# Soltanilara/av-aloha

Hardware: AMD Instinct MI355X
Metric: env-steps/sec (whole node) at 4096 parallel envs, SlotInsertion-3Arms (higher is better)
Workload: dtype f32

## Files before the change

### av_aloha_amd/csrc/avsim_phys.hip.h

```cpp
#pragma once
#include <hip/hip_runtime.h>

#include <cstddef>
#include <cstring>
#include <string>
#include <type_traits>
#include <vector>

#include "avsim_collide.hip.h"
#include "avsim_dev.h"
#include "avsim_math.hip.h"
#include "avsim_model.h"
#include "avsim_phys_layout.h"

namespace avs {

enum { J_FREE = 0, J_BALL = 1, J_SLIDE = 2, J_HINGE = 3 };
enum { R_EQ = 0, R_FLOSS = 1, R_LIMIT = 2, R_CONTACT = 3 };
constexpr int TREE_W = 8;
constexpr int ROW_W = 2 * TREE_W;
constexpr int ROW_S = ROW_W;
constexpr int CAND_MAX = 256;
constexpr int PROF_W = 26;
constexpr int NEAR_MAX = 512;
// ... 277 lines not shown
    const long long b = __builtin_bit_cast(long long, x);
    const unsigned lo = (unsigned)__builtin_amdgcn_readlane((int)(unsigned)b, l), hi = (unsigned)__builtin_amdgcn_readlane((int)(unsigned)(b >> 32), l);
    return __builtin_bit_cast(double, ((long long)hi << 32) | (long long)lo);
}

constexpr int GRP_MAX = 6;
constexpr int GA_W = 64, GA_Q = 16, GA_QW = 6;
template <typename T> AVS_DEV T qdiv(T t, T d, T dinv) { return sizeof(T) == 4 ? t * dinv : t / d; }
AVS_DEV float qrsqrt(float x) { return __builtin_amdgcn_rsqf(x); }
AVS_DEV double qrsqrt(double x) { return 1.0 / sqrt(x); }
template <typename T> struct QTol;
template <> struct QTol<double> { static constexpr double abs = 1e-10, rel = 0.0; };
template <> struct QTol<float> { static constexpr float abs = 1e-10f, rel = 2e-6f; };

template <bool B> struct BoolTag { static constexpr bool value = B; };

template <typename real>
struct NoslipLead {
    LDS_PTR(const real) Minv;
    LDS_PTR(const int) tadr;
    LDS_PTR(const int) tnum;
    LDS_PTR(const int) floss_dof;
    LDS_PTR(int) dmap;
    LDS_PTR(int) prof;
    int tridiag;
    int ntree, nv, neq, nfloss, nlg;
};

typedef int nl_v4 __attribute__((ext_vector_type(4)));
#define NL_PARAMS nl_v4 nl_a_, nl_v4 nl_b_, nl_v4 nl_c_
// ... 1277 lines not shown
    }
    int l = latch ? latch[i] : 0;
    reward[i] = reward_from_flags(f, task_id, &l);
    if (latch) latch[i] = l;
}
#endif


template <typename real, int G, typename SPEC = GenericSpec>
struct Env {
    KRef<real, SPEC> ka;
    int env = 0;
    int diverged = 0;
    int nit_sum = 0, nit_max = 0;
    bool profiling = false;
    real* r;
    int* ii;
    int lane, grp;
    const real* lr;
    const int* li;
    long long t_broad = 0, t_narrow = 0;
    __device__ Env(KRef<real, SPEC> ka_, real* r_, int* i_, int lane_, int grp_, const real* lr_, const int* li_)
        : ka(ka_), r(r_), ii(i_), lane(lane_), grp(grp_), lr(lr_), li(li_) {}
    AVS_DEV const int* LI() const {
        const int* p = li;
        if constexpr (spec_fixed<SPEC>) p = lds_at<const int>((unsigned)(ka->mo.nreal * sizeof(real)));
        AVS_ASSUME_LDS(p);
        return p;
    }
    AVS_DEV const real* LR() const {
        const real* p = lr;
        if constexpr (spec_fixed<SPEC>) p = lds_at<const real>(0u);
        AVS_ASSUME_LDS(p);
        return p;
    }
    AVS_DEV int nobj_() const { if constexpr (spec_fixed<SPEC>) return SPEC::nobj; else return ka->m.nobj; }
    AVS_DEV int hull_ovf_() const { if constexpr (spec_fixed<SPEC>) return SPEC::hull_ovf; else return ka->m.hull_ovf; }
    AVS_DEV GArr<real> rows_() const { return glb_block((GLB_PTR(real))ka->m.rJ_glob, env, (unsigned)(ka->lay.gefc * ROW_S)); }
    AVS_DEV GArr<real> rowsB_() const { return glb_block((GLB_PTR(real))ka->m.rB_glob, env, (unsigned)(ka->lay.gefc * ROW_S)); }
    AVS_DEV GArr<real> coup_() const { return glb_block((GLB_PTR(real))ka->m.gA_glob, env, (unsigned)(ka->lay.ggrp * GA_W)); }
    AVS_DEV GArr<int> near_() const { return glb_block((GLB_PTR(int))ka->m.near_glob, env, (unsigned)NEAR_MAX); }
    AVS_DEV GArr<int> cand_() const { return glb_block((GLB_PTR(int))ka->m.cand_glob, env, (unsigned)CAND_MAX); }
    AVS_DEV GArr<real> bxo_() const { return glb_block((GLB_PTR(real))ka->m.bxo_glob, env, (unsigned)(64 * BOX_OVF_W)); }
    AVS_DEV GArr<real> gref_() const { return glb_block((GLB_PTR(real))ka->m.gref_glob, env, (unsigned)(ka->m.ngeom * 3)); }
    AVS_DEV const int* body_parent_() const { return LI() + ka->mo.body_parent; }
    AVS_DEV const int* body_jntadr_() const { return LI() + ka->mo.body_jntadr; }
    AVS_DEV const int* body_jntnum_() const { return LI() + ka->mo.body_jntnum; }
    AVS_DEV const int* body_dofadr_() const { return LI() + ka->mo.body_dofadr; }
    AVS_DEV const int* body_dofnum_() const { return LI() + ka->mo.body_dofnum; }
    AVS_DEV const int* body_tree_() const { return LI() + ka->mo.body_tree; }
    AVS_DEV const int* body_dofmask_() const { return LI() + ka->mo.body_dofmask; }
    AVS_DEV const int* body_last_() const { return LI() + ka->mo.body_last; }
// ... 737 lines not shown
            nefc += tot;
        }
        nefc = cend;
        if (lane == 0) { misc[1] = nefc; if (ovf) misc[2] |= 2; }
        GSYNC();
        ROWPROBE(0);
        const GArr<real> rJ = rows_();
        real *rowS = r + ka->lay.rowS, *warm = r + ka->lay.warm, *Minv = r + ka->lay.Minv, *asm_ = r + ka->lay.asm_;
        const bool newton = ka->m.solver == 1;
        const bool lead_slim = newton && lead_per_tree();
        int* rowI = ii + ka->lay.rowI;
        real* Lm = r + ka->lay.L;
        const int *bmask = body_dofmask_(), *tadr = tree_dofadr_(), *tnum = tree_dofnum_();
        const real* cdofp = r + ka->lay.cdof;
        const int nvm = ka->m.nv - 1;
        auto fill = [&](int i, auto lead_tag) {
            constexpr bool LEAD = decltype(lead_tag)::value;
            int meta = rmeta[i], type = meta & 3, id = (meta >> 2) & 1023, sub = (meta >> 12) & 255, dim = meta >> 20;
            real J[ROW_W];
#pragma unroll
            for (int k = 0; k < ROW_W; k++) J[k] = 0;
            int tA = -1, tB = -1;
            int j1 = -1, j2 = -1;
            real v1 = 0, v2 = 0;
            real pos = 0, margin = 0, diag0 = 0, floss = 0;
            real solref[2], solimp[5];
            bool valid = true;
            if (LEAD && type == R_EQ) {
                const GArr<const real> c = TAB(eq_polycoef) + 5 * id;
                real q1 = qpos[TAB(eq_qpos1)[id]] - TAB(qpos0)[TAB(eq_qpos1)[id]], q2 = qpos[TAB(eq_qpos2)[id]] - TAB(qpos0)[TAB(eq_qpos2)[id]];
                real poly = c[0] + q2 * (c[1] + q2 * (c[2] + q2 * (c[3] + q2 * c[4])));
                real dpoly = c[1] + q2 * (2 * c[2] + q2 * (3 * c[3] + q2 * 4 * c[4]));
                int d1 = TAB(eq_dof1)[id], d2 = TAB(eq_dof2)[id];
                tA = dof_tree_()[d1];
                pos = q1 - poly;
                diag0 = dof_invweight0_()[d1] + dof_invweight0_()[d2];
                j1 = d1 - tree_dofadr_()[tA]; v1 = 1;
                j2 = d2 - tree_dofadr_()[tA]; v2 = -dpoly;
                for (int k = 0; k < 2; k++) solref[k] = (TAB(eq_solref) + 2 * id)[k];
                for (int k = 0; k < 5; k++) solimp[k] = (TAB(eq_solimp) + 5 * id)[k];
            } else if (LEAD && type == R_FLOSS) {
                int d = floss_dof_()[id];
                tA = dof_tree_()[d];
                diag0 = dof_invweight0_()[d];
                floss = dof_frictionloss_()[d];
                j1 = d - tree_dofadr_()[tA]; v1 = 1;
                for (int k = 0; k < 2; k++) solref[k] = (TAB(dof_solref) + 2 * d)[k];
                for (int k = 0; k < 5; k++) solimp[k] = (TAB(dof_solimp) + 5 * d)[k];
            } else if (LEAD && type == R_LIMIT) {
                int j = id, d = jnt_dofadr_()[j];
                real q = qpos[jnt_qposadr_()[j]];
                tA = dof_tree_()[d];
                pos = sub == 0 ? q - jnt_range_()[2 * j] : jnt_range_()[2 * j + 1] - q;
                margin = jnt_margin_()[j];
                diag0 = dof_invweight0_()[d];
                j1 = d - tree_dofadr_()[tA]; v1 = sub == 0 ? real(1) : real(-1);
                for (int k = 0; k < 2; k++) solref[k] = (TAB(jnt_solref) + 2 * j)[k];
                for (int k = 0; k < 5; k++) solimp[k] = (TAB(jnt_solimp) + 5 * j)[k];
            } else if (!LEAD) {
                int c = id, p = cpair[c];
                int g1 = (TAB(pair_geom) + 2 * p)[0], g2 = (TAB(pair_geom) + 2 * p)[1], b1 = geom_body_()[g1], b2 = geom_body_()[g2];
                int t1 = body_tree_()[b1], t2 = body_tree_()[b2];
                tA = t1 >= 0 ? t1 : t2;
                tB = (t1 >= 0 && t2 >= 0 && t2 != t1) ? t2 : -1;
                real n[3] = {cnrm[3 * c], cnrm[3 * c + 1], cnrm[3 * c + 2]}, t1v[3], t2v[3], cp[3] = {cpos[3 * c], cpos[3 * c + 1], cpos[3 * c + 2]};
                make_frame(n, t1v, t2v);
                const int sm = sub % 3;
                real ax[3];
#pragma unroll
                for (int q = 0; q < 3; q++) ax[q] = sm == 0 ? n[q] : (sm == 1 ? t1v[q] : t2v[q]);
                const bool rot = sub >= 3;
                real cx[3], Wa[3], Wl[3];
                cross3(cp, ax, cx);
#pragma unroll
                for (int q = 0; q < 3; q++) { Wa[q] = rot ? ax[q] : cx[q]; Wl[q] = rot ? real(0) : ax[q]; }
                const int mA = (t1 == tA ? bmask[b1] : 0), pA = (t2 == tA ? bmask[b2] : 0);
                const int mB = (tB >= 0 && t1 == tB ? bmask[b1] : 0), pB = (tB >= 0 ? bmask[b2] : 0);
                const int aA = tadr[tA], aB = tadr[tB >= 0 ? tB : tA];
#pragma unroll
                for (int k = 0; k < TREE_W; k++) {
                    const real* ca = cdofp + 6 * (aA + k < nvm ? aA + k : nvm);
                    const real ea = Wa[0] * ca[0] + Wa[1] * ca[1] + Wa[2] * ca[2] + Wl[0] * ca[3] + Wl[1] * ca[4] + Wl[2] * ca[5];
                    J[k] = real(((pA >> k) & 1) - ((mA >> k) & 1)) * ea;
                }
                if (tB >= 0) {
#pragma unroll
                    for (int k = 0; k < TREE_W; k++) {
                        const real* cb = cdofp + 6 * (aB + k < nvm ? aB + k : nvm);
                        const real eb = Wa[0] * cb[0] + Wa[1] * cb[1] + Wa[2] * cb[2] + Wl[0] * cb[3] + Wl[1] * cb[4] + Wl[2] * cb[5];
                        J[TREE_W + k] = real(((pB >> k) & 1) - ((mB >> k) & 1)) * eb;
                    }
                }
                pos = sub == 0 ? cdist[c] : real(0);
                margin = TAB(pair_margin)[p] - TAB(pair_gap)[p];
                diag0 = body_invweight0_()[2 * b1] + body_invweight0_()[2 * b2];
                for (int k = 0; k < 2; k++) solref[k] = (TAB(pair_solref) + 2 * p)[k];
                for (int k = 0; k < 5; k++) solimp[k] = (TAB(pair_solimp) + 5 * p)[k];
            }
            (void)valid;
            const int j2c = j2 >= 0 ? j2 : (j1 >= 0 ? j1 : 0), j1c = j1 >= 0 ? j1 : 0;
            const real v2c = j2 >= 0 ? v2 : real(0);
            if (LEAD) {
#pragma unroll
                for (int k = 0; k < TREE_W; k++) J[k] += (k == j1 ? v1 : real(0)) + (k == j2 ? v2 : real(0));
            }
            real dmax = tclamp(solimp[1], real(0.0001), real(0.9999));
            real tc = tmax(solref[0], 2 * ka->m.timestep), dr = solref[1];
            real K = real(1) / tmax(real(1e-15), dmax * dmax * tc * tc * dr * dr), Bd = real(2) / tmax(real(1e-15), dmax * tc);
            real imp, R;
            const real imp_row = impedance(solimp, (!LEAD && sub > 0) ? cdist[id] : pos, margin);
            if (!LEAD && sub > 0) {
                int c = id, p = cpair[c];
                real imp0 = imp_row;
                real R0 = tmax(real(1e-15), (1 - imp0) * diag0 / imp0);
                real R1 = R0 / tmax(real(1e-15), ka->m.impratio);
                real mu0 = (TAB(pair_friction) + 5 * p)[0], mur = (TAB(pair_friction) + 5 * p)[sub - 1];
                R = sub == 1 ? R1 : R1 * mu0 * mu0 / tmax(real(1e-15), mur * mur);
                imp = imp0;
                K = 0;
                floss = mur;
            } else {
                imp = imp_row;
                R = tmax(real(1e-15), (1 - imp) * diag0 / imp);
            }
            real vel = 0;
            if (LEAD) {
                const int a0 = tadr[tA];
                vel = v1 * qvel[a0 + j1c] + v2c * qvel[a0 + j2c];
            } else {
                const int a0 = tadr[tA], b0 = tadr[tB >= 0 ? tB : tA];
#pragma unroll
                for (int k = 0; k < TREE_W; k++) vel += J[k] * qvel[a0 + k < nvm ? a0 + k : nvm];
                if (tB >= 0) {
#pragma unroll
                    for (int k = 0; k < TREE_W; k++) vel += J[TREE_W + k] * qvel[b0 + k < nvm ? b0 + k : nvm];
                }
            }
            const real aref = -Bd * vel - K * imp * (pos - margin);
            real dg = 0;
            real Bv[ROW_W];
            if (LEAD) {
                const real* Mi = Minv + 64 * tA;
                const real s1 = Mi[8 * j1c + j1c] * v1 + Mi[8 * j1c + j2c] * v2c, s2 = Mi[8 * j2c + j1c] * v1 + Mi[8 * j2c + j2c] * v2c;
                dg = v1 * s1 + v2c * s2;
                if (!lead_slim) {
#pragma unroll
                    for (int k = 0; k < TREE_W; k++) { Bv[k] = Mi[8 * k + j1c] * v1 + Mi[8 * k + j2c] * v2c; Bv[TREE_W + k] = 0; }
                }
            } else {
#pragma unroll
            for (int k = 0; k < TREE_W; k++) {
                real mr[TREE_W], sa = 0;
                lds_load8(Minv + 64 * tA + 8 * k, mr);
#pragma unroll
                for (int j = 0; j < TREE_W; j++) sa += mr[j] * J[j];
                dg += J[k] * sa;
                Bv[k] = sa;
                Bv[TREE_W + k] = 0;
            }
            if (tB >= 0) {
#pragma unroll
                for (int k = 0; k < TREE_W; k++) {
                    real mr[TREE_W], sb = 0;
                    lds_load8(Minv + 64 * tB + 8 * k, mr);
#pragma unroll
                    for (int j = 0; j < TREE_W; j++) sb += mr[j] * J[TREE_W + j];
                    dg += J[TREE_W + k] * sb;
                    Bv[TREE_W + k] = sb;
                }
            }
            }
            if (!LEAD && tB < 0) {
                real JB_[ROW_W];
#pragma unroll
                for (int k = 0; k < TREE_W; k++) { JB_[k] = J[k]; JB_[TREE_W + k] = Bv[k]; }
                store_row16(rJ + ROW_S * i, JB_);
            } else if (!LEAD || !lead_slim) {
                store_row16(rJ + ROW_S * i, J);
                store_row16(rowsB_() + ROW_S * i, Bv);
            }
            const int a0 = tadr[tA], nA = tnum[tA], b0 = tB >= 0 ? tadr[tB] : 0, nB = tB >= 0 ? tnum[tB] : 0;
            real jw = 0, jas = 0;
            if (LEAD) {
                jw = v1 * warm[a0 + j1c] + v2c * warm[a0 + j2c];
                jas = v1 * asm_[a0 + j1c] + v2c * asm_[a0 + j2c];
            } else {
#pragma unroll
            for (int k = 0; k < TREE_W; k++) {
                const int da = a0 + k < nvm ? a0 + k : nvm;
                jw += J[k] * warm[da];
                jas += J[k] * asm_[da];
            }
            if (tB >= 0) {
#pragma unroll
                for (int k = 0; k < TREE_W; k++) {
                    const int db = b0 + k < nvm ? b0 + k : nvm;
                    jw += J[TREE_W + k] * warm[db];
                    jas += J[TREE_W + k] * asm_[db];
                }
            }
            }
            const real big = real(1e30);
            real lo = -big, hi = big, muinv = 0;
            bool ns = false;
            if (LEAD && type == R_FLOSS) { lo = -floss; hi = floss; ns = true; }
            else if (LEAD && type == R_LIMIT) lo = 0;
            else if (!LEAD) {
                if (sub == 0) lo = 0;
                else { ns = true; muinv = real(1) / tmax(real(1e-15), floss); }
            }
            real f = -(jw - aref) / R;
            f = tmin(tmax(f, lo), hi);
            real* S = rowS + RS_S * i;
            S[0] = aref; S[1] = R; S[2] = newton ? jw - aref : real(1) / (dg + R); S[3] = ns ? real(1) / tmax(dg, real(1e-15)) : real(0);
            S[4] = lo; S[5] = hi; S[6] = f; S[7] = muinv; S[8] = jas - aref;
            const int lead_bits = !LEAD ? 0 : ((v1 < 0 ? 1 : 0) << 13) | (j1c << 26) | (j2c << 29);
            if (LEAD) S[7] = v2c;
            rowI[i] = a0 | (nA << 6) | (tA << 10) | ((b0 | (nB << 6) | ((tB >= 0 ? tB : 0) << 10)) << 13) | lead_bits;
            rmeta[i] = (meta & 0xfffff) | ((tA + 1) << 20) | ((tB + 1) << 24);
        };
        for (int i = lane; i < nlead0; i += G) fill(i, BoolTag<true>{});
        ROWPROBE(1);
        for (int i = nlead0 + lane; i < nefc; i += G) fill(i, BoolTag<false>{});
        GSYNC();
        ROWPROBE(2);
        int* gI = ii + ka->lay.gI;
        const GArr<real> gA = coup_();
        const int nlead = misc[4];
        int ngrp = 0;
        for (int base = 0; base < nefc; base += G) {
            int i = base + lane;
            bool head = false;
            int cnt = 0, isc = 0;
            if (i < nefc) {
                if (i < nlead) { head = (i % GRP_MAX) == 0; cnt = nlead - i < GRP_MAX ? nlead - i : GRP_MAX; }
                else { int meta = rmeta[i]; head = ((meta >> 12) & 255) == 0; cnt = TAB(pair_condim)[cpair[(meta >> 2) & 1023]]; isc = 1; }
            }
            int tot, rk = group_rank<G>(head, grp, lane, &tot);
// ... 369 lines not shown
    }
    KRef<real, SPEC> ka = (RETRY && big) ? ka_big : ka_small;
    const long long t_launch = __builtin_readcyclecounter();
    real* r = reinterpret_cast<real*>(smem + rec0 + (size_t)((RETRY && big) ? (wave & ~1) : wave) * ka_small->lay.bytes_per_env);
    int* ii = reinterpret_cast<int*>(r + ka->lay.nreal);
    bool beyond = false;
    Env<real, G, SPEC> E(ka, r, ii, lane, grp, lr, li);
    E.env = env;

    for (int i = lane; i < ka->m.nq; i += G) r[ka->lay.qpos + i] = g_qpos[(size_t)env * ka->m.nq + i];
    for (int i = lane; i < ka->m.nv; i += G) { r[ka->lay.qvel + i] = g_qvel[(size_t)env * ka->m.nv + i]; r[ka->lay.warm + i] = g_warm[(size_t)env * ka->m.nv + i]; }
    for (int i = lane; i < ka->m.nu; i += G) r[ka->lay.ctrl + i] = g_ctrl[(size_t)env * ka->m.nu + i];
    if (lane == 0) for (int k = 0; k < 8; k++) { ii[ka->lay.misc + k] = 0; ii[ka->lay.nprof + k] = 0; ii[ka->lay.nprof + 8 + k] = 0; }
    if (lane == 0) ii[ka->lay.misc + 8] = 0;
    E.profiling = o_prof != nullptr;
    GSYNC();
    if (action) {
        const float* a = action + (size_t)env * ka->m.nj;
        for (int i = lane; i < ka->m.nj; i += G) {
            real v = (real)a[i];
            if (i == 6 || i == 13) v = v * (ka->m.grip_hi - ka->m.grip_lo) + ka->m.grip_lo;
            r[ka->lay.ctrl + i] = v;
        }
        GSYNC();
    }
    long long tp[9] = {0, 0, 0, 0, 0, 0, 0, 0, 0};
#define PROF(k, stmt) do { if (o_prof) { long long t0_ = __builtin_readcyclecounter(); stmt; tp[k] += __builtin_readcyclecounter() - t0_; } else { stmt; } } while (0)
    for (int s = 0; s < nsub; s++) {
#ifndef AVS_NO_SPLIT_PRE
        PROF(0, E.pre_phases());
// ... 105 lines not shown
    __syncthreads();
    if (threadIdx.x == 0) { int a = 0; for (int b = 0; b < 256; b++) { off[b] = a; a += cnt[b]; } }
    __syncthreads();
    for (int i = threadIdx.x; i < N; i += 1024) order[atomicAdd(&off[bucket(cost[i])], 1)] = i;
}

struct PhysHost;
int phys_launch_f64(PhysHost& ph, hipStream_t st, int nsub, const float* action, void* qpos, void* qvel, void* ctrl, void* warm, int* latch,
                    double* agent, int32_t* reward, uint8_t* success, std::string& err);
const void* phys_spec_kernel(const PhysHost& ph, const char** name);

struct PhysHost {
    int maxcon = 48, maxefc = 144, pgs_iters = 20, group = 64, export_contacts = 1, force_reward = 0, wpb_override = 0;
    int maxcon1 = 48, maxefc1 = 144;
    bool f64 = false;
    int specialised = 1;
    bool host_only = false;
    int N = 0, max_reward = 0;
    DevArena arena;
    DevModel<float> mf;
    DevModel<double> md;
    Layout lay, lay2;
    bool two_pass() const { return maxcon1 < maxcon || maxefc1 < maxefc; }
    int pair_waves = 1;
    int* d_retry = nullptr;
    unsigned long long retry_parity = 0;
    DevBuf kargs2;
    double *d_qpos_home = nullptr, *d_ctrl_home = nullptr, *d_obj_reset = nullptr;
    int* d_obj_qadr = nullptr;
    int *d_ncon = nullptr, *d_diag = nullptr;
// ... 234 lines not shown
            m.hull_vert = upr<real>(tab);
        }
        m.pair_geom = up(I("pair_geom")); m.pair_condim = up(I("pair_condim"));
        m.pair_friction = upr<real>(F("pair_friction")); m.pair_solref = upr<real>(F("pair_solref")); m.pair_solimp = upr<real>(F("pair_solimp"));
        m.pair_margin = upr<real>(F("pair_margin")); m.pair_gap = upr<real>(F("pair_gap"));
        m.obs_qposadr = up(I("obs_qposadr")); m.obs_offset = upr<real>(F("obs_offset")); m.obs_scale = upr<real>(F("obs_scale"));
        while (img_real.size() % 4) img_real.push_back(0.0);
        while (img_int.size() % 4) img_int.push_back(0);
        moff.nreal = (int)img_real.size();
        moff.nint = (int)img_int.size();
        d_img_real = (void*)upr<real>(img_real);
        d_img_int = up(img_int);
    }

    const void* spec_kernel(const char** name) const {
        if (f64 || specialised == 0 || two_pass()) return nullptr;
        return phys_spec_kernel(*this, name);
    }
    bool refuses(std::string& err) const {
        if (specialised != 2 || spec_kernel(nullptr)) return false;
        err = std::string("phys_specialised = 2: no kernel compiled for this handle's model and layout (") +
              (f64 ? "f64 handle" : two_pass() ? "two capacity tiers" : "Layout, table offsets, dims or solver options (solver, noslip_*, qcqp_tridiag, newton_*, ls_iterations, num_joints) match no spec of avsim_phys_specs.h") + "); the launch would take the generic k_phys";
        return true;
    }
    int spec_note = 0;

    void make_layout(int nq, int nv, int nu, int nb, int ng, int msize, int ntree) {
        if (maxcon1 > maxcon) maxcon1 = maxcon;
        if (maxefc1 > maxefc) maxefc1 = maxefc;
        make_layout_of(lay, maxcon1, maxefc1, nq, nv, nu, nb, ng, msize, ntree);
        make_layout_of(lay2, maxcon, maxefc, nq, nv, nu, nb, ng, msize, ntree);
    }
    void make_layout_of(Layout& L, const int maxcon, const int maxefc, int nq, int nv, int nu, int nb, int ng, int msize, int ntree) {
        kargs_dirty = true;
        L = avs::make_layout_of(maxcon, maxefc, this->maxcon, this->maxefc, nq, nv, nu, nb, ng, msize, ntree, f64 ? 8 : 4);
        if (getenv("AVSIM_DEBUG_LAYOUT")) {
            const int pb = L.rowS + RS_S * maxefc > L.scr + NARROW_SCR_W ? L.rowS + RS_S * maxefc : L.scr + NARROW_SCR_W;
// ... 55 lines not shown
    }
    bool set_option(const char* name, double v) {
        std::string n(name);
        kargs_dirty = true;
        if (n == "pgs_iters") { pgs_iters = (int)v; return true; }
        if (n == "solver") { if (v != 0 && v != 1) return false; mf.solver = md.solver = (int)v; return true; }
        if (n == "newton_iters") { if (v < 1 || v > 100) return false; mf.newton_iters = md.newton_iters = (int)v; return true; }
        if (n == "newton_tol") { if (v < 0) return false; mf.newton_tol = (float)v; md.newton_tol = v; return true; }
        if (n == "ls_tolerance") { if (!(v > 0) || v >= 1) return false; mf.ls_tolerance = (float)v; md.ls_tolerance = v; return true; }
        if (n == "ls_iterations") { if (v < 1 || v > 1000) return false; mf.ls_iterations = md.ls_iterations = (int)v; return true; }
        if (n == "export_contacts") { export_contacts = v != 0; return true; }
        if (n == "num_joints") { if (v != 14 && v != 21) return false; mf.nj = md.nj = (int)v; return true; }
        if (n == "order_envs") { order_envs = v != 0; return true; }
        if (n == "phys_specialised") { if (v != 0 && v != 1 && v != 2) return false; specialised = (int)v; return true; }
        if (n == "pair_waves") { pair_waves = v != 0; return true; }
        if (n == "qcqp_tridiag") { mf.qcqp_tridiag = md.qcqp_tridiag = v < 0 ? 0 : (v > 2 ? 2 : (int)v); return true; }
        if (n == "noslip_iters") { if (v < 0 || v > 100) return false; mf.noslip_iters = md.noslip_iters = (int)v; return true; }
        if (n == "noslip_per_tree") { mf.noslip_per_tree = md.noslip_per_tree = v != 0; return true; }
        if (n == "noslip_trees") { mf.noslip_trees = md.noslip_trees = v != 0; return true; }
        if (n == "newton_component") { mf.newton_component = md.newton_component = v != 0; return true; }
        if (n == "newton_early_exit") { mf.newton_early_exit = md.newton_early_exit = v != 0; return true; }
        if (n == "persist_blocks") { int x = (int)v; if (x >= 1 && x <= 64) { persist_over = x; return true; } return false; }
        if (n == "waves_per_block") { int x = (int)v; if (x >= 0 && x <= AVSIM_PHYS_MAXW) { wpb_override = x; return true; } return false; }
        if (n == "profile_phases") {
            if (v != 0 && !d_prof) d_prof = up(std::vector<long long>((size_t)N * PROF_W, 0));
            if (v == 0) d_prof = nullptr;
            return true;
        }
        if (n == "maxefc" || n == "maxcon" || n == "maxefc_first" || n == "maxcon_first") {
            int x = (int)v;
// ... 57 lines not shown
        if (!two && wpb_override <= 0 && num_cu > 0 && N < num_cu * wpb) { wpb = (N + num_cu - 1) / num_cu; if (wpb < 1) wpb = 1; }
        const size_t pairflags = two ? 2 * (MAXW / 2 > 0 ? MAXW / 2 : 1) * sizeof(int) : 0;
        const size_t shmem = (size_t)lay.bytes_per_env * wpb + tables + pairflags, shmem2 = (size_t)lay2.bytes_per_env * wpb2 + tables + pairflags;
        const int pairing = (two && wpb >= 2 && lay2.bytes_per_env <= 2 * lay.bytes_per_env && pair_waves) ? 8 : 0;
        if (shmem > 160 * 1024 || (two && shmem2 > 160 * 1024)) { err = "per-block LDS exceeds 160 KiB; lower maxefc/maxcon"; return -1; }
        const int per_cu = (int)((160 * 1024) / shmem) > 0 ? (int)((160 * 1024) / shmem) : 1;
        int nblk = num_cu * per_cu * (persist_over > 0 ? persist_over : 1);
        if (nblk > (N + wpb - 1) / wpb) nblk = (N + wpb - 1) / wpb;
        if (kargs_dirty) {
            KArgs<real> ka{m, lay, moff}, ka2{m, lay2, moff};
            if (kargs.reserve(sizeof(KArgs<double>)) != hipSuccess || kargs2.reserve(sizeof(KArgs<double>)) != hipSuccess) { err = "hipMalloc(kernel arguments) failed"; return -3; }
            (void)hipStreamSynchronize(st);
            if (hipMemcpy(kargs.ptr(), &ka, sizeof(ka), hipMemcpyHostToDevice) != hipSuccess || hipMemcpy(kargs2.ptr(), &ka2, sizeof(ka2), hipMemcpyHostToDevice) != hipSuccess) { err = "hipMemcpy(kernel arguments) failed"; return -3; }
            kargs_dirty = false;
        }
        static_assert((8 | 7) < (1 << 8), "retry_mode: mode bits and pairing flag below bit 8");
        if (two && (maxcon1 >= 1024 || maxefc1 >= 1024 || maxcon1 < 0 || maxefc1 < 0)) { err = "first-tier capacities do not fit the 10-bit fields of retry_mode (maxcon_first / maxefc_first < 1024)"; return -1; }
        const int* order = nullptr;
        if (order_envs && have_cost && nsub > 0 && N > wpb) {
            hipLaunchKernelGGL(k_env_order, dim3(1), dim3(1024), 0, st, (const int*)d_cost, d_order, N);
            order = d_order;
        }
        const int want_reward = (reward || success) && (nsub > 0 || force_reward) ? 1 : 0;
        const int par = (int)(retry_parity & 1);
        int* const rlist = d_retry + 2;
        {
            int* head = this->head.as<int>() + (launch_count & 1);
            int* next = this->head.as<int>() + ((launch_count + 1) & 1);
            launch_count++;
            hipLaunchKernelGGL(two ? kern2 : kern1, dim3(nblk), dim3(64 * wpb), shmem, st, (KPtr<real>)kargs.ptr(), (const real*)d_img_real, (const int*)d_img_int, N, nsub, pgs_iters, action, want_reward,
                               (real*)qpos, (real*)qvel, (real*)ctrl, (real*)warm, latch, agent, (int*)reward, (unsigned char*)success, d_ncon,
                               cpairs.as<int>(), cdist.as<double>(), d_diag, max_reward, export_contacts, d_prof, d_xpose, order, order_envs ? d_cost : (int*)nullptr, head, next,
                               d_retry, two ? (1 + 2 * par) | pairing : 0, (KPtr<real>)kargs2.ptr());
        }
        if (two) {
            int* head = this->head.as<int>() + (launch_count & 1);
            int* next = this->head.as<int>() + ((launch_count + 1) & 1);
            launch_count++;
            retry_parity++;
            int nblk2 = num_cu;
            if (nblk2 > (N + wpb2 - 1) / wpb2) nblk2 = (N + wpb2 - 1) / wpb2;
            hipLaunchKernelGGL(kern2, dim3(nblk2), dim3(64 * wpb2), shmem2, st, (KPtr<real>)kargs2.ptr(), (const real*)d_img_real, (const int*)d_img_int, N, nsub, pgs_iters, action, want_reward,
                               (real*)qpos, (real*)qvel, (real*)ctrl, (real*)warm, latch, agent, (int*)reward, (unsigned char*)success, d_ncon,
                               cpairs.as<int>(), cdist.as<double>(), d_diag, max_reward, export_contacts, d_prof, d_xpose, (const int*)rlist, order_envs ? d_cost : (int*)nullptr, head, next,
                               d_retry, (2 + 2 * par) | (maxcon1 << 8) | (maxefc1 << 18), (KPtr<real>)kargs2.ptr());
        }
        if (nsub > 0) have_cost = true;
        hipError_t e = hipGetLastError();
        if (e != hipSuccess) { err = std::string("physics kernel launch: ") + hipGetErrorString(e); return -3; }
        return 0;
    }

#if !defined(AVSIM_TU_F64) && !defined(AVSIM_NO_F32_LAUNCH)
    int launch(hipStream_t st, int N_, int nsub, const float* action, int nj, void* qpos, void* qvel, void* ctrl, void* warm, int* latch,
               double* agent, int32_t* reward, uint8_t* success, std::string& err) {
        (void)N_; (void)nj;
        if (f64) return phys_launch_f64(*this, st, nsub, action, qpos, qvel, ctrl, warm, latch, agent, reward, success, err);
        return launch_t<float, 64, AVSIM_PHYS_MAXW>(st, mf, nsub, action, qpos, qvel, ctrl, warm, latch, agent, reward, success, err);
    }
#endif
// ... 20 lines not shown
```

### av_aloha_amd/csrc/avsim_phys_layout.h

```cpp
#pragma once

namespace avs {

constexpr int RS_S = 9;
constexpr int ANC_MAX = 64;
constexpr int NARROW_SCR_W = 64 * 24 + 4 * 56;

struct MOff {
    int nreal, nint;
    int body_parent;
    int body_jntadr;
    int body_jntnum;
    int body_dofadr;
    int body_dofnum;
    int body_tree;
    int body_dofmask;
    int body_last;
    int tree_bodyadr;
    int tree_bodylist;
    int tree_dofadr;
    int tree_dofnum;
    int tree_madr;
    int jnt_type;
    int jnt_qposadr;
// ... 80 lines not shown
    L.cand = io; io += ANC_MAX; L.cpair = io; io += maxcon; L.cefc = io; io += maxcon; L.rmeta = io; io += maxefc; L.rowI = io; io += maxefc;
    L.gI = io; io += maxefc / 3 + 8; L.misc = io; io += 12; L.nprof = io; io += 16;
    L.nint = (io + 3) & ~3;
    L.maxcon = maxcon;
    L.maxefc = maxefc;
    L.expcon = full_maxcon;
    L.gefc = full_maxefc;
    L.ggrp = full_maxefc / 3 + 8;
    L.bytes_per_env = (int)(((unsigned long long)L.nreal * (unsigned)real_bytes + (unsigned long long)L.nint * 4 + 15) & ~15ull);
    return L;
}

constexpr int CAP_EFC[5] = {176, 176, 336, 480, 176}, CAP_CON[5] = {48, 48, 72, 96, 48};
constexpr int CAP_EFC1[5] = {176, 176, 224, 288, 176}, CAP_CON1[5] = {48, 48, 56, 64, 48};

}
```

Baseline: 1.057 million.

## Fill contact constraint rows in axis pairs sharing per-contact setup

Splits the row-fill lambda into a lead-row path and a contact path. The contact path can compute two rows per lane, one translational and one rotational along the same axis, so the contact frame, pair lookups and cdof loads are shared between them. It is used when a per-lane pairing over 3*ncon items needs fewer wavefront trips than one row per lane. The paired mode is on by default and can be turned off with a rows_paired option that falls back to the generic kernel. The cost is more registers per lane from the doubled J arrays, which could lower occupancy.

```diff
diff --git a/av_aloha_amd/csrc/avsim_phys.hip.h b/av_aloha_amd/csrc/avsim_phys.hip.h
--- a/av_aloha_amd/csrc/avsim_phys.hip.h
+++ b/av_aloha_amd/csrc/avsim_phys.hip.h
@@ -315,6 +315,7 @@
 template <> struct QTol<float> { static constexpr float abs = 1e-10f, rel = 2e-6f; };
 
 template <bool B> struct BoolTag { static constexpr bool value = B; };
+template <int I> struct IntTag { static constexpr int value = I; };
 
 template <typename real>
 struct NoslipLead {
@@ -1622,6 +1623,7 @@
     int diverged = 0;
     int nit_sum = 0, nit_max = 0;
     bool profiling = false;
+    bool rows_single = false;
     real* r;
     int* ii;
     int lane, grp;
@@ -1644,6 +1646,7 @@
     }
     AVS_DEV int nobj_() const { if constexpr (spec_fixed<SPEC>) return SPEC::nobj; else return ka->m.nobj; }
     AVS_DEV int hull_ovf_() const { if constexpr (spec_fixed<SPEC>) return SPEC::hull_ovf; else return ka->m.hull_ovf; }
+    AVS_DEV bool rows_paired_() const { if constexpr (spec_fixed<SPEC>) return true; else return !rows_single; }
     AVS_DEV GArr<real> rows_() const { return glb_block((GLB_PTR(real))ka->m.rJ_glob, env, (unsigned)(ka->lay.gefc * ROW_S)); }
     AVS_DEV GArr<real> rowsB_() const { return glb_block((GLB_PTR(real))ka->m.rB_glob, env, (unsigned)(ka->lay.gefc * ROW_S)); }
     AVS_DEV GArr<real> coup_() const { return glb_block((GLB_PTR(real))ka->m.gA_glob, env, (unsigned)(ka->lay.ggrp * GA_W)); }
@@ -2411,19 +2414,17 @@
         const int *bmask = body_dofmask_(), *tadr = tree_dofadr_(), *tnum = tree_dofnum_();
         const real* cdofp = r + ka->lay.cdof;
         const int nvm = ka->m.nv - 1;
-        auto fill = [&](int i, auto lead_tag) {
-            constexpr bool LEAD = decltype(lead_tag)::value;
-            int meta = rmeta[i], type = meta & 3, id = (meta >> 2) & 1023, sub = (meta >> 12) & 255, dim = meta >> 20;
+        auto fill_lead = [&](int i) {
+            int meta = rmeta[i], type = meta & 3, id = (meta >> 2) & 1023, sub = (meta >> 12) & 255;
             real J[ROW_W];
 #pragma unroll
             for (int k = 0; k < ROW_W; k++) J[k] = 0;
-            int tA = -1, tB = -1;
+            int tA = -1;
             int j1 = -1, j2 = -1;
             real v1 = 0, v2 = 0;
             real pos = 0, margin = 0, diag0 = 0, floss = 0;
             real solref[2], solimp[5];
-            bool valid = true;
-            if (LEAD && type == R_EQ) {
+            if (type == R_EQ) {
                 const GArr<const real> c = TAB(eq_polycoef) + 5 * id;
                 real q1 = qpos[TAB(eq_qpos1)[id]] - TAB(qpos0)[TAB(eq_qpos1)[id]], q2 = qpos[TAB(eq_qpos2)[id]] - TAB(qpos0)[TAB(eq_qpos2)[id]];
                 real poly = c[0] + q2 * (c[1] + q2 * (c[2] + q2 * (c[3] + q2 * c[4])));
@@ -2436,7 +2437,7 @@
                 j2 = d2 - tree_dofadr_()[tA]; v2 = -dpoly;
                 for (int k = 0; k < 2; k++) solref[k] = (TAB(eq_solref) + 2 * id)[k];
                 for (int k = 0; k < 5; k++) solimp[k] = (TAB(eq_solimp) + 5 * id)[k];
-            } else if (LEAD && type == R_FLOSS) {
+            } else if (type == R_FLOSS) {
                 int d = floss_dof_()[id];
                 tA = dof_tree_()[d];
                 diag0 = dof_invweight0_()[d];
@@ -2444,7 +2445,7 @@
                 j1 = d - tree_dofadr_()[tA]; v1 = 1;
                 for (int k = 0; k < 2; k++) solref[k] = (TAB(dof_solref) + 2 * d)[k];
                 for (int k = 0; k < 5; k++) solimp[k] = (TAB(dof_solimp) + 5 * d)[k];
-            } else if (LEAD && type == R_LIMIT) {
+            } else if (type == R_LIMIT) {
                 int j = id, d = jnt_dofadr_()[j];
                 real q = qpos[jnt_qposadr_()[j]];
                 tA = dof_tree_()[d];
@@ -2454,171 +2455,243 @@
                 j1 = d - tree_dofadr_()[tA]; v1 = sub == 0 ? real(1) : real(-1);
                 for (int k = 0; k < 2; k++) solref[k] = (TAB(jnt_solref) + 2 * j)[k];
                 for (int k = 0; k < 5; k++) solimp[k] = (TAB(jnt_solimp) + 5 * j)[k];
-            } else if (!LEAD) {
-                int c = id, p = cpair[c];
-                int g1 = (TAB(pair_geom) + 2 * p)[0], g2 = (TAB(pair_geom) + 2 * p)[1], b1 = geom_body_()[g1], b2 = geom_body_()[g2];
-                int t1 = body_tree_()[b1], t2 = body_tree_()[b2];
-                tA = t1 >= 0 ? t1 : t2;
-                tB = (t1 >= 0 && t2 >= 0 && t2 != t1) ? t2 : -1;
-                real n[3] = {cnrm[3 * c], cnrm[3 * c + 1], cnrm[3 * c + 2]}, t1v[3], t2v[3], cp[3] = {cpos[3 * c], cpos[3 * c + 1], cpos[3 * c + 2]};
-                make_frame(n, t1v, t2v);
-                const int sm = sub % 3;
-                real ax[3];
-#pragma unroll
-                for (int q = 0; q < 3; q++) ax[q] = sm == 0 ? n[q] : (sm == 1 ? t1v[q] : t2v[q]);
-                const bool rot = sub >= 3;
-                real cx[3], Wa[3], Wl[3];
-                cross3(cp, ax, cx);
-#pragma unroll
-                for (int q = 0; q < 3; q++) { Wa[q] = rot ? ax[q] : cx[q]; Wl[q] = rot ? real(0) : ax[q]; }
-                const int mA = (t1 == tA ? bmask[b1] : 0), pA = (t2 == tA ? bmask[b2] : 0);
-                const int mB = (tB >= 0 && t1 == tB ? bmask[b1] : 0), pB = (tB >= 0 ? bmask[b2] : 0);
-                const int aA = tadr[tA], aB = tadr[tB >= 0 ? tB : tA];
-#pragma unroll
-                for (int k = 0; k < TREE_W; k++) {
-                    const real* ca = cdofp + 6 * (aA + k < nvm ? aA + k : nvm);
-                    const real ea = Wa[0] * ca[0] + Wa[1] * ca[1] + Wa[2] * ca[2] + Wl[0] * ca[3] + Wl[1] * ca[4] + Wl[2] * ca[5];
-                    J[k] = real(((pA >> k) & 1) - ((mA >> k) & 1)) * ea;
-                }
-                if (tB >= 0) {
-#pragma unroll
-                    for (int k = 0; k < TREE_W; k++) {
-                        const real* cb = cdofp + 6 * (aB + k < nvm ? aB + k : nvm);
-                        const real eb = Wa[0] * cb[0] + Wa[1] * cb[1] + Wa[2] * cb[2] + Wl[0] * cb[3] + Wl[1] * cb[4] + Wl[2] * cb[5];
-                        J[TREE_W + k] = real(((pB >> k) & 1) - ((mB >> k) & 1)) * eb;
-                    }
-                }
-                pos = sub == 0 ? cdist[c] : real(0);
-                margin = TAB(pair_margin)[p] - TAB(pair_gap)[p];
-                diag0 = body_invweight0_()[2 * b1] + body_invweight0_()[2 * b2];
-                for (int k = 0; k < 2; k++) solref[k] = (TAB(pair_solref) + 2 * p)[k];
-                for (int k = 0; k < 5; k++) solimp[k] = (TAB(pair_solimp) + 5 * p)[k];
-            }
-            (void)valid;
+            }
             const int j2c = j2 >= 0 ? j2 : (j1 >= 0 ? j1 : 0), j1c = j1 >= 0 ? j1 : 0;
             const real v2c = j2 >= 0 ? v2 : real(0);
-            if (LEAD) {
-#pragma unroll
-                for (int k = 0; k < TREE_W; k++) J[k] += (k == j1 ? v1 : real(0)) + (k == j2 ? v2 : real(0));
-            }
+#pragma unroll
+            for (int k = 0; k < TREE_W; k++) J[k] += (k == j1 ? v1 : real(0)) + (k == j2 ? v2 : real(0));
             real dmax = tclamp(solimp[1], real(0.0001), real(0.9999));
             real tc = tmax(solref[0], 2 * ka->m.timestep), dr = solref[1];
             real K = real(1) / tmax(real(1e-15), dmax * dmax * tc * tc * dr * dr), Bd = real(2) / tmax(real(1e-15), dmax * tc);
-            real imp, R;
-            const real imp_row = impedance(solimp, (!LEAD && sub > 0) ? cdist[id] : pos, margin);
-            if (!LEAD && sub > 0) {
-                int c = id, p = cpair[c];
-                real imp0 = imp_row;
-                real R0 = tmax(real(1e-15), (1 - imp0) * diag0 / imp0);
-                real R1 = R0 / tmax(real(1e-15), ka->m.impratio);
-                real mu0 = (TAB(pair_friction) + 5 * p)[0], mur = (TAB(pair_friction) + 5 * p)[sub - 1];
-                R = sub == 1 ? R1 : R1 * mu0 * mu0 / tmax(real(1e-15), mur * mur);
-                imp = imp0;
-                K = 0;
-                floss = mur;
-            } else {
-                imp = imp_row;
-                R = tmax(real(1e-15), (1 - imp) * diag0 / imp);
-            }
-            real vel = 0;
-            if (LEAD) {
-                const int a0 = tadr[tA];
-                vel = v1 * qvel[a0 + j1c] + v2c * qvel[a0 + j2c];
-            } else {
-                const int a0 = tadr[tA], b0 = tadr[tB >= 0 ? tB : tA];
-#pragma unroll
-                for (int k = 0; k < TREE_W; k++) vel += J[k] * qvel[a0 + k < nvm ? a0 + k : nvm];
-                if (tB >= 0) {
-#pragma unroll
-                    for (int k = 0; k < TREE_W; k++) vel += J[TREE_W + k] * qvel[b0 + k < nvm ? b0 + k : nvm];
-                }
-            }
+            const real imp = impedance(solimp, pos, margin);
+            const real R = tmax(real(1e-15), (1 - imp) * diag0 / imp);
+            const int a0 = tadr[tA], nA = tnum[tA];
+            const real vel = v1 * qvel[a0 + j1c] + v2c * qvel[a0 + j2c];
             const real aref = -Bd * vel - K * imp * (pos - margin);
-            real dg = 0;
-            real Bv[ROW_W];
-            if (LEAD) {
-                const real* Mi = Minv + 64 * tA;
-                const real s1 = Mi[8 * j1c + j1c] * v1 + Mi[8 * j1c + j2c] * v2c, s2 = Mi[8 * j2c + j1c] * v1 + Mi[8 * j2c + j2c] * v2c;
-                dg = v1 * s1 + v2c * s2;
-                if (!lead_slim) {
-#pragma unroll
-                    for (int k = 0; k < TREE_W; k++) { Bv[k] = Mi[8 * k + j1c] * v1 + Mi[8 * k + j2c] * v2c; Bv[TREE_W + k] = 0; }
-                }
-            } else {
-#pragma unroll
-            for (int k = 0; k < TREE_W; k++) {
-                real mr[TREE_W], sa = 0;
-                lds_load8(Minv + 64 * tA + 8 * k, mr);
-#pragma unroll
-                for (int j = 0; j < TREE_W; j++) sa += mr[j] * J[j];
-                dg += J[k] * sa;
-                Bv[k] = sa;
-                Bv[TREE_W + k] = 0;
-            }
-            if (tB >= 0) {
-#pragma unroll
-                for (int k = 0; k < TREE_W; k++) {
-                    real mr[TREE_W], sb = 0;
-                    lds_load8(Minv + 64 * tB + 8 * k, mr);
-#pragma unroll
-                    for (int j = 0; j < TREE_W; j++) sb += mr[j] * J[TREE_W + j];
-                    dg += J[TREE_W + k] * sb;
-                    Bv[TREE_W + k] = sb;
-                }
-            }
-            }
-            if (!LEAD && tB < 0) {
-                real JB_[ROW_W];
-#pragma unroll
-                for (int k = 0; k < TREE_W; k++) { JB_[k] = J[k]; JB_[TREE_W + k] = Bv[k]; }
-                store_row16(rJ + ROW_S * i, JB_);
-            } else if (!LEAD || !lead_slim) {
+            const real* Mi = Minv + 64 * tA;
+            const real s1 = Mi[8 * j1c + j1c] * v1 + Mi[8 * j1c + j2c] * v2c, s2 = Mi[8 * j2c + j1c] * v1 + Mi[8 * j2c + j2c] * v2c;
+            const real dg = v1 * s1 + v2c * s2;
+            if (!lead_slim) {
+                real Bv[ROW_W];
+#pragma unroll
+                for (int k = 0; k < TREE_W; k++) { Bv[k] = Mi[8 * k + j1c] * v1 + Mi[8 * k + j2c] * v2c; Bv[TREE_W + k] = 0; }
                 store_row16(rJ + ROW_S * i, J);
                 store_row16(rowsB_() + ROW_S * i, Bv);
             }
-            const int a0 = tadr[tA], nA = tnum[tA], b0 = tB >= 0 ? tadr[tB] : 0, nB = tB >= 0 ? tnum[tB] : 0;
-            real jw = 0, jas = 0;
-            if (LEAD) {
-                jw = v1 * warm[a0 + j1c] + v2c * warm[a0 + j2c];
-                jas = v1 * asm_[a0 + j1c] + v2c * asm_[a0 + j2c];
-            } else {
-#pragma unroll
-            for (int k = 0; k < TREE_W; k++) {
-                const int da = a0 + k < nvm ? a0 + k : nvm;
-                jw += J[k] * warm[da];
-                jas += J[k] * asm_[da];
-            }
-            if (tB >= 0) {
-#pragma unroll
-                for (int k = 0; k < TREE_W; k++) {
-                    const int db = b0 + k < nvm ? b0 + k : nvm;
-                    jw += J[TREE_W + k] * warm[db];
-                    jas += J[TREE_W + k] * asm_[db];
-                }
-            }
-            }
+            const real jw = v1 * warm[a0 + j1c] + v2c * warm[a0 + j2c];
+            const real jas = v1 * asm_[a0 + j1c] + v2c * asm_[a0 + j2c];
             const real big = real(1e30);
-            real lo = -big, hi = big, muinv = 0;
+            real lo = -big, hi = big;
             bool ns = false;
-            if (LEAD && type == R_FLOSS) { lo = -floss; hi = floss; ns = true; }
-            else if (LEAD && type == R_LIMIT) lo = 0;
-            else if (!LEAD) {
-                if (sub == 0) lo = 0;
-                else { ns = true; muinv = real(1) / tmax(real(1e-15), floss); }
-            }
+            if (type == R_FLOSS) { lo = -floss; hi = floss; ns = true; }
+            else if (type == R_LIMIT) lo = 0;
             real f = -(jw - aref) / R;
             f = tmin(tmax(f, lo), hi);
             real* S = rowS + RS_S * i;
             S[0] = aref; S[1] = R; S[2] = newton ? jw - aref : real(1) / (dg + R); S[3] = ns ? real(1) / tmax(dg, real(1e-15)) : real(0);
-            S[4] = lo; S[5] = hi; S[6] = f; S[7] = muinv; S[8] = jas - aref;
-            const int lead_bits = !LEAD ? 0 : ((v1 < 0 ? 1 : 0) << 13) | (j1c << 26) | (j2c << 29);
-            if (LEAD) S[7] = v2c;
-            rowI[i] = a0 | (nA << 6) | (tA << 10) | ((b0 | (nB << 6) | ((tB >= 0 ? tB : 0) << 10)) << 13) | lead_bits;
-            rmeta[i] = (meta & 0xfffff) | ((tA + 1) << 20) | ((tB + 1) << 24);
+            S[4] = lo; S[5] = hi; S[6] = f; S[8] = jas - aref;
+            S[7] = v2c;
+            rowI[i] = a0 | (nA << 6) | (tA << 10) | ((v1 < 0 ? 1 : 0) << 13) | (j1c << 26) | (j2c << 29);
+            rmeta[i] = (meta & 0xfffff) | ((tA + 1) << 20);
         };
-        for (int i = lane; i < nlead0; i += G) fill(i, BoolTag<true>{});
+        auto fill_con = [&](const int c, const int i0, const int sub0, const bool live1, auto nr_tag) {
+            constexpr int NR = decltype(nr_tag)::value;
+            const int p = cpair[c];
+            const int g1 = (TAB(pair_geom) + 2 * p)[0], g2 = (TAB(pair_geom) + 2 * p)[1], b1 = geom_body_()[g1], b2 = geom_body_()[g2];
+            const int t1 = body_tree_()[b1], t2 = body_tree_()[b2];
+            const int tA = t1 >= 0 ? t1 : t2;
+            const int tB = (t1 >= 0 && t2 >= 0 && t2 != t1) ? t2 : -1;
+            real n[3] = {cnrm[3 * c], cnrm[3 * c + 1], cnrm[3 * c + 2]}, t1v[3], t2v[3], cp[3] = {cpos[3 * c], cpos[3 * c + 1], cpos[3 * c + 2]};
+            make_frame(n, t1v, t2v);
+            const int mA = (t1 == tA ? bmask[b1] : 0), pA = (t2 == tA ? bmask[b2] : 0);
+            const int mB = (tB >= 0 && t1 == tB ? bmask[b1] : 0), pB = (tB >= 0 ? bmask[b2] : 0);
+            const int a0 = tadr[tA], b0 = tadr[tB >= 0 ? tB : tA];
+            const real margin = TAB(pair_margin)[p] - TAB(pair_gap)[p];
+            const real diag0 = body_invweight0_()[2 * b1] + body_invweight0_()[2 * b2];
+            real solref[2], solimp[5];
+            for (int k = 0; k < 2; k++) solref[k] = (TAB(pair_solref) + 2 * p)[k];
+            for (int k = 0; k < 5; k++) solimp[k] = (TAB(pair_solimp) + 5 * p)[k];
+            int sub[NR];
+            real J[NR][ROW_W];
+            real Wa[NR][3], Wl[NR][3];
+#pragma unroll
+            for (int q = 0; q < NR; q++) {
+                sub[q] = sub0 + 3 * q;
+#pragma unroll
+                for (int k = 0; k < ROW_W; k++) J[q][k] = 0;
+                const int sm = sub[q] % 3;
+                real ax[3];
+#pragma unroll
+                for (int x = 0; x < 3; x++) ax[x] = sm == 0 ? n[x] : (sm == 1 ? t1v[x] : t2v[x]);
+                const bool rot = sub[q] >= 3;
+                real cx[3];
+                cross3(cp, ax, cx);
+#pragma unroll
+                for (int x = 0; x < 3; x++) { Wa[q][x] = rot ? ax[x] : cx[x]; Wl[q][x] = rot ? real(0) : ax[x]; }
+            }
+#pragma unroll
+            for (int k = 0; k < TREE_W; k++) {
+                const real* ca = cdofp + 6 * (a0 + k < nvm ? a0 + k : nvm);
+#pragma unroll
+                for (int q = 0; q < NR; q++) {
+                    const real ea = Wa[q][0] * ca[0] + Wa[q][1] * ca[1] + Wa[q][2] * ca[2] + Wl[q][0] * ca[3] + Wl[q][1] * ca[4] + Wl[q][2] * ca[5];
+                    J[q][k] = real(((pA >> k) & 1) - ((mA >> k) & 1)) * ea;
+                }
+            }
+            if (tB >= 0) {
+#pragma unroll
+                for (int k = 0; k < TREE_W; k++) {
+                    const real* cb = cdofp + 6 * (b0 + k < nvm ? b0 + k : nvm);
+#pragma unroll
+                    for (int q = 0; q < NR; q++) {
+                        const real eb = Wa[q][0] * cb[0] + Wa[q][1] * cb[1] + Wa[q][2] * cb[2] + Wl[q][0] * cb[3] + Wl[q][1] * cb[4] + Wl[q][2] * cb[5];
+                        J[q][TREE_W + k] = real(((pB >> k) & 1) - ((mB >> k) & 1)) * eb;
+                    }
+                }
+            }
+            asm volatile("" : "+v"(solimp[0]), "+v"(solimp[1]), "+v"(solimp[2]), "+v"(solimp[3]), "+v"(solimp[4]), "+v"(solref[0]), "+v"(solref[1]));
+            const real dmax = tclamp(solimp[1], real(0.0001), real(0.9999));
+            const real tc = tmax(solref[0], 2 * ka->m.timestep), dr = solref[1];
+            const real K0 = real(1) / tmax(real(1e-15), dmax * dmax * tc * tc * dr * dr), Bd = real(2) / tmax(real(1e-15), dmax * tc);
+            const real imp = impedance(solimp, cdist[c], margin);
+            const real R0 = tmax(real(1e-15), (1 - imp) * diag0 / imp);
+            const real R1 = R0 / tmax(real(1e-15), ka->m.impratio);
+            const real mu0 = (TAB(pair_friction) + 5 * p)[0];
+            real R[NR], K[NR], floss[NR], pos[NR];
+#pragma unroll
+            for (int q = 0; q < NR; q++) {
+                pos[q] = sub[q] == 0 ? cdist[c] : real(0);
+                R[q] = R0; K[q] = K0; floss[q] = 0;
+                if (sub[q] > 0) {
+                    const real mur = (TAB(pair_friction) + 5 * p)[sub[q] - 1];
+                    R[q] = sub[q] == 1 ? R1 : R1 * mu0 * mu0 / tmax(real(1e-15), mur * mur);
+                    K[q] = 0;
+                    floss[q] = mur;
+                }
+            }
+            real vel[NR];
+#pragma unroll
+            for (int q = 0; q < NR; q++) {
+                vel[q] = 0;
+#pragma unroll
+                for (int k = 0; k < TREE_W; k++) vel[q] += J[q][k] * qvel[a0 + k < nvm ? a0 + k : nvm];
+            }
+            if (tB >= 0) {
+#pragma unroll
+                for (int q = 0; q < NR; q++) {
+#pragma unroll
+                    for (int k = 0; k < TREE_W; k++) vel[q] += J[q][TREE_W + k] * qvel[b0 + k < nvm ? b0 + k : nvm];
+                }
+            }
+            real aref[NR];
+#pragma unroll
+            for (int q = 0; q < NR; q++) aref[q] = -Bd * vel[q] - K[q] * imp * (pos[q] - margin);
+            real dg[NR];
+            real Bv[NR][ROW_W];
+#pragma unroll
+            for (int q = 0; q < NR; q++) dg[q] = 0;
+#pragma unroll
+            for (int k = 0; k < TREE_W; k++) {
+                real mr[TREE_W];
+                lds_load8(Minv + 64 * tA + 8 * k, mr);
+#pragma unroll
+                for (int q = 0; q < NR; q++) {
+                    real sa = 0;
+#pragma unroll
+                    for (int j = 0; j < TREE_W; j++) sa += mr[j] * J[q][j];
+                    dg[q] += J[q][k] * sa;
+                    Bv[q][k] = sa;
+                    Bv[q][TREE_W + k] = 0;
+                }
+            }
+            if (tB >= 0) {
+#pragma unroll
+                for (int k = 0; k < TREE_W; k++) {
+                    real mr[TREE_W];
+                    lds_load8(Minv + 64 * tB + 8 * k, mr);
+#pragma unroll
+                    for (int q = 0; q < NR; q++) {
+                        real sb = 0;
+#pragma unroll
+                        for (int j = 0; j < TREE_W; j++) sb += mr[j] * J[q][TREE_W + j];
+                        dg[q] += J[q][TREE_W + k] * sb;
+                        Bv[q][TREE_W + k] = sb;
+                    }
+                }
+            }
+            if (tB < 0) {
+#pragma unroll
+                for (int q = 0; q < NR; q++) {
+                    real JB_[ROW_W];
+#pragma unroll
+                    for (int k = 0; k < TREE_W; k++) { JB_[k] = J[q][k]; JB_[TREE_W + k] = Bv[q][k]; }
+                    if (q == 0 || live1) store_row16(rJ + ROW_S * (i0 + 3 * q), JB_);
+                }
+            } else {
+#pragma unroll
+                for (int q = 0; q < NR; q++)
+                    if (q == 0 || live1) {
+                        store_row16(rJ + ROW_S * (i0 + 3 * q), J[q]);
+                        store_row16(rowsB_() + ROW_S * (i0 + 3 * q), Bv[q]);
+                    }
+            }
+            const int nA = tnum[tA], b0r = tB >= 0 ? tadr[tB] : 0, nB = tB >= 0 ? tnum[tB] : 0;
+            real jw[NR], jas[NR];
+#pragma unroll
+            for (int q = 0; q < NR; q++) {
+                jw[q] = 0; jas[q] = 0;
+#pragma unroll
+                for (int k = 0; k < TREE_W; k++) {
+                    const int da = a0 + k < nvm ? a0 + k : nvm;
+                    jw[q] += J[q][k] * warm[da];
+                    jas[q] += J[q][k] * asm_[da];
+                }
+            }
+            if (tB >= 0) {
+#pragma unroll
+                for (int q = 0; q < NR; q++) {
+#pragma unroll
+                    for (int k = 0; k < TREE_W; k++) {
+                        const int db = b0r + k < nvm ? b0r + k : nvm;
+                        jw[q] += J[q][TREE_W + k] * warm[db];
+                        jas[q] += J[q][TREE_W + k] * asm_[db];
+                    }
+                }
+            }
+            const real big = real(1e30);
+#pragma unroll
+            for (int q = 0; q < NR; q++) {
+                const int i = i0 + 3 * q;
+                real lo = -big, hi = big, muinv = 0;
+                bool ns = false;
+                if (sub[q] == 0) lo = 0;
+                else { ns = true; muinv = real(1) / tmax(real(1e-15), floss[q]); }
+                real f = -(jw[q] - aref[q]) / R[q];
+                f = tmin(tmax(f, lo), hi);
+                if (q == 0 || live1) {
+                    real* S = rowS + RS_S * i;
+                    S[0] = aref[q]; S[1] = R[q]; S[2] = newton ? jw[q] - aref[q] : real(1) / (dg[q] + R[q]); S[3] = ns ? real(1) / tmax(dg[q], real(1e-15)) : real(0);
+                    S[4] = lo; S[5] = hi; S[6] = f; S[7] = muinv; S[8] = jas[q] - aref[q];
+                    rowI[i] = a0 | (nA << 6) | (tA << 10) | ((b0r | (nB << 6) | ((tB >= 0 ? tB : 0) << 10)) << 13);
+                    rmeta[i] = R_CONTACT | (c << 2) | (sub[q] << 12) | ((tA + 1) << 20) | ((tB + 1) << 24);
+                }
+            }
+        };
+        for (int i = lane; i < nlead0; i += G) fill_lead(i);
         ROWPROBE(1);
-        for (int i = nlead0 + lane; i < nefc; i += G) fill(i, BoolTag<false>{});
+        if (rows_paired_() && rows_pair_pays(ncon, nefc - nlead0, G)) {
+            for (int base = 0; base < 3 * ncon; base += G) {
+                const int item = base + lane, c = item / 3, s = item - 3 * c;
+                int row0 = 0;
+                bool live1 = false;
+                if (axis_rows(c < ncon ? cefc[c] : -1, s, row0, live1)) fill_con(c, row0, s, live1, IntTag<2>{});
+            }
+        } else {
+            for (int i = nlead0 + lane; i < nefc; i += G) {
+                const int meta = rmeta[i];
+                fill_con((meta >> 2) & 1023, i, (meta >> 12) & 255, false, IntTag<1>{});
+            }
+        }
         GSYNC();
         ROWPROBE(2);
         int* gI = ii + ka->lay.gI;
@@ -3018,6 +3091,7 @@
     if (lane == 0) for (int k = 0; k < 8; k++) { ii[ka->lay.misc + k] = 0; ii[ka->lay.nprof + k] = 0; ii[ka->lay.nprof + 8 + k] = 0; }
     if (lane == 0) ii[ka->lay.misc + 8] = 0;
     E.profiling = o_prof != nullptr;
+    E.rows_single = (retry_mode & 16) != 0;
     GSYNC();
     if (action) {
         const float* a = action + (size_t)env * ka->m.nj;
@@ -3153,6 +3227,7 @@
     int maxcon = 48, maxefc = 144, pgs_iters = 20, group = 64, export_contacts = 1, force_reward = 0, wpb_override = 0;
     int maxcon1 = 48, maxefc1 = 144;
     bool f64 = false;
+    int rows_paired = 1;
     int specialised = 1;
     bool host_only = false;
     int N = 0, max_reward = 0;
@@ -3417,13 +3492,13 @@
     }
 
     const void* spec_kernel(const char** name) const {
-        if (f64 || specialised == 0 || two_pass()) return nullptr;
+        if (f64 || specialised == 0 || two_pass() || !rows_paired) return nullptr;
         return phys_spec_kernel(*this, name);
     }
     bool refuses(std::string& err) const {
         if (specialised != 2 || spec_kernel(nullptr)) return false;
         err = std::string("phys_specialised = 2: no kernel compiled for this handle's model and layout (") +
-              (f64 ? "f64 handle" : two_pass() ? "two capacity tiers" : "Layout, table offsets, dims or solver options (solver, noslip_*, qcqp_tridiag, newton_*, ls_iterations, num_joints) match no spec of avsim_phys_specs.h") + "); the launch would take the generic k_phys";
+              (f64 ? "f64 handle" : two_pass() ? "two capacity tiers" : !rows_paired ? "rows_paired = 0" :"Layout, table offsets, dims or solver options (solver, noslip_*, qcqp_tridiag, newton_*, ls_iterations, num_joints) match no spec of avsim_phys_specs.h") + "); the launch would take the generic k_phys";
         return true;
     }
     int spec_note = 0;
@@ -3509,6 +3584,7 @@
         if (n == "order_envs") { order_envs = v != 0; return true; }
         if (n == "phys_specialised") { if (v != 0 && v != 1 && v != 2) return false; specialised = (int)v; return true; }
         if (n == "pair_waves") { pair_waves = v != 0; return true; }
+        if (n == "rows_paired") { if (v != 0 && v != 1) return false; rows_paired = (int)v; return true; }
         if (n == "qcqp_tridiag") { mf.qcqp_tridiag = md.qcqp_tridiag = v < 0 ? 0 : (v > 2 ? 2 : (int)v); return true; }
         if (n == "noslip_iters") { if (v < 0 || v > 100) return false; mf.noslip_iters = md.noslip_iters = (int)v; return true; }
         if (n == "noslip_per_tree") { mf.noslip_per_tree = md.noslip_per_tree = v != 0; return true; }
@@ -3596,7 +3672,8 @@
             if (hipMemcpy(kargs.ptr(), &ka, sizeof(ka), hipMemcpyHostToDevice) != hipSuccess || hipMemcpy(kargs2.ptr(), &ka2, sizeof(ka2), hipMemcpyHostToDevice) != hipSuccess) { err = "hipMemcpy(kernel arguments) failed"; return -3; }
             kargs_dirty = false;
         }
-        static_assert((8 | 7) < (1 << 8), "retry_mode: mode bits and pairing flag below bit 8");
+        static_assert((16 | 8 | 7) < (1 << 8), "retry_mode: mode bits, pairing flag and the rows_paired = 0 flag below bit 8");
+        const int single = rows_paired ? 0 : 16;
         if (two && (maxcon1 >= 1024 || maxefc1 >= 1024 || maxcon1 < 0 || maxefc1 < 0)) { err = "first-tier capacities do not fit the 10-bit fields of retry_mode (maxcon_first / maxefc_first < 1024)"; return -1; }
         const int* order = nullptr;
         if (order_envs && have_cost && nsub > 0 && N > wpb) {
@@ -3613,7 +3690,7 @@
             hipLaunchKernelGGL(two ? kern2 : kern1, dim3(nblk), dim3(64 * wpb), shmem, st, (KPtr<real>)kargs.ptr(), (const real*)d_img_real, (const int*)d_img_int, N, nsub, pgs_iters, action, want_reward,
                                (real*)qpos, (real*)qvel, (real*)ctrl, (real*)warm, latch, agent, (int*)reward, (unsigned char*)success, d_ncon,
                                cpairs.as<int>(), cdist.as<double>(), d_diag, max_reward, export_contacts, d_prof, d_xpose, order, order_envs ? d_cost : (int*)nullptr, head, next,
-                               d_retry, two ? (1 + 2 * par) | pairing : 0, (KPtr<real>)kargs2.ptr());
+                               d_retry, (two ? (1 + 2 * par) | pairing : 0) | single, (KPtr<real>)kargs2.ptr());
         }
         if (two) {
             int* head = this->head.as<int>() + (launch_count & 1);
@@ -3625,7 +3702,7 @@
             hipLaunchKernelGGL(kern2, dim3(nblk2), dim3(64 * wpb2), shmem2, st, (KPtr<real>)kargs2.ptr(), (const real*)d_img_real, (const int*)d_img_int, N, nsub, pgs_iters, action, want_reward,
                                (real*)qpos, (real*)qvel, (real*)ctrl, (real*)warm, latch, agent, (int*)reward, (unsigned char*)success, d_ncon,
                                cpairs.as<int>(), cdist.as<double>(), d_diag, max_reward, export_contacts, d_prof, d_xpose, (const int*)rlist, order_envs ? d_cost : (int*)nullptr, head, next,
-                               d_retry, (2 + 2 * par) | (maxcon1 << 8) | (maxefc1 << 18), (KPtr<real>)kargs2.ptr());
+                               d_retry, (2 + 2 * par) | single | (maxcon1 << 8) | (maxefc1 << 18), (KPtr<real>)kargs2.ptr());
         }
         if (nsub > 0) have_cost = true;
         hipError_t e = hipGetLastError();
diff --git a/av_aloha_amd/csrc/avsim_phys_layout.h b/av_aloha_amd/csrc/avsim_phys_layout.h
--- a/av_aloha_amd/csrc/avsim_phys_layout.h
+++ b/av_aloha_amd/csrc/avsim_phys_layout.h
@@ -118,4 +118,14 @@
 constexpr int CAP_EFC[5] = {176, 176, 336, 480, 176}, CAP_CON[5] = {48, 48, 72, 96, 48};
 constexpr int CAP_EFC1[5] = {176, 176, 224, 288, 176}, CAP_CON1[5] = {48, 48, 56, 64, 48};
 
+constexpr int row_trips(int n, int lanes) { return (n + lanes - 1) / lanes; }
+constexpr bool rows_pair_pays(int ncon, int ncontact_rows, int lanes) { return row_trips(3 * ncon, lanes) < row_trips(ncontact_rows, lanes); }
+constexpr bool axis_rows(int ce, int s, int& row0, bool& live1) {
+    const int first = ce & 0xffff, dim = ce >> 16;
+    if (ce < 0 || s >= dim) return false;
+    row0 = first + s;
+    live1 = s + 3 < dim;
+    return true;
 }
+
+}
```

After: 1.069 million (median of 6 runs). 1.0% higher.
